# korrawe/harp

Measured on AMD Instinct MI355X. Metric: render+loss+backward+Adam frames/sec, 512x512 MANO hand mesh, higher is better.
Workload: dtype f32; 1 GPU; C3/C4: 256-frame 512x512 sequence, subdivided MANO hand 3093v/6152f/3327uv, self-shadow, coarse+appearance terms (displacement+texture stage, VGG excluded), dense Adam; global_batch=32, sequence_frames=256, hipgraph=True

## Files before the change

### harp_amd/csrc/raster.hip

```cpp
#include <stdlib.h>
#include <mutex>
#include <unordered_map>
#include "raster_body.h"

namespace {

using rb::Tri;

template <bool BITS>
__device__ __forceinline__ void face_setup_body(const float* __restrict__ ndc, const int32_t* __restrict__ faces,
                                                int V, int F, float r, FaceRec* __restrict__ recs,
                                                float4* __restrict__ bbs, int S, int nsx, unsigned long long* __restrict__ bits, int W64) {
  const int f = blockIdx.x * blockDim.x + threadIdx.x;
  const int b = blockIdx.y;
  float4 bb = make_float4(3.0e38f, -3.0e38f, 3.0e38f, -3.0e38f);
  if (f < F) {
    const FaceRec rec = rb::face_rec(ndc + (size_t)b * V * 3, faces, f, r);
    recs[(size_t)b * F + f] = rec;
    bbs[(size_t)b * F + f] = rec.bb;
    bb = rec.bb;
  }
  if constexpr (BITS) {
    const int lane = threadIdx.x & 63;
    const int chunk = f >> 6;
// ... 24 lines not shown
  face_setup_body<BITS>(ndc, faces, V, F, r, recs, bbs, S, nsx, bits, W64);
}

struct SetupView { const float* ndc; float r; RasterWs W; };

__global__ void __launch_bounds__(256) face_setup_pair_kernel(const SetupView a, const SetupView b, const int32_t* __restrict__ faces, int V, int F, int S) {
  const SetupView& v = blockIdx.z ? b : a;
  face_setup_body<true>(v.ndc, faces, V, F, v.r, v.W.recs, v.W.bbs, S, v.W.nsx, v.W.bits, v.W.W64);
}

__global__ void __launch_bounds__(256) bin_faces_kernel(const float4* __restrict__ bbs, int F, int S, int nsx,
                                                        int32_t* __restrict__ bins, int32_t* __restrict__ bin_count) {
  const int nst = nsx * nsx;
  const int st = blockIdx.x * 4 + (threadIdx.x >> 6), b = blockIdx.y;
  if (st >= nst) return;
  rb::bin_super_tile(bbs + (size_t)b * F, F, S, nsx, st, bins + ((size_t)b * nst + st) * F, bin_count + b * nst + st);
}

__device__ __forceinline__ void expand_bits_body(const unsigned long long* __restrict__ bits, int F, int W64, int nst,
                                                 int32_t* __restrict__ bins, int32_t* __restrict__ bin_count) {
  const int st = blockIdx.x * 4 + (threadIdx.x >> 6), b = blockIdx.y, lane = threadIdx.x & 63;
  if (st >= nst) return;
  const unsigned long long* src = bits + ((size_t)b * nst + st) * W64;
  int32_t* out = bins + ((size_t)b * nst + st) * F;
  int total = 0;
  for (int base = 0; base < W64; base += 128) {
    unsigned long long w0 = (base + lane < W64) ? src[base + lane] : 0ull;
    unsigned long long w1 = (base + 64 + lane < W64) ? src[base + 64 + lane] : 0ull;
    const int c0 = __popcll(w0), c1 = __popcll(w1);
    int incl = c0 | (c1 << 16);
#pragma unroll
    for (int o = 1; o < 64; o <<= 1) {
      const int t = __shfl_up(incl, o, 64);
      if (lane >= o) incl += t;
    }
    const int tot = __shfl(incl, 63, 64);
    int pos = total + (incl & 0xffff) - c0;
    const int f0 = (base + lane) * 64;
    while (w0) {
      out[pos++] = f0 + (int)__builtin_ctzll(w0);
      w0 &= w0 - 1ull;
    }
    pos = total + (tot & 0xffff) + (incl >> 16) - c1;
    while (w1) {
      out[pos++] = f0 + 4096 + (int)__builtin_ctzll(w1);
      w1 &= w1 - 1ull;
    }
    total += (tot & 0xffff) + (tot >> 16);
  }
  if (lane == 0) bin_count[b * nst + st] = total;
}
__global__ void __launch_bounds__(256) expand_bits_kernel(const unsigned long long* __restrict__ bits, int F, int W64, int nst,
                                                          int32_t* __restrict__ bins, int32_t* __restrict__ bin_count) {
  expand_bits_body(bits, F, W64, nst, bins, bin_count);
}
__global__ void __launch_bounds__(256) expand_bits_pair_kernel(const RasterWs a, const RasterWs b, int F) {
  const RasterWs& W = blockIdx.z ? b : a;
  expand_bits_body(W.bits, F, W.W64, W.nsx * W.nsx, W.bins, W.cnt);
}

__global__ void __launch_bounds__(1024) order_tiles_kernel(const int32_t* __restrict__ bin_count, int total, int32_t* __restrict__ order,
                                                           int32_t* __restrict__ nact) {
  __shared__ int s_hist[33], s_base[33];
  rb::order_tiles(bin_count, total, order, nact, s_hist, s_base);
}

__global__ void __launch_bounds__(1024) order_tiles_pair_kernel(const RasterWs a, const RasterWs b, int total) {
  __shared__ int s_hist[33], s_base[33];
  const RasterWs& W = blockIdx.x ? b : a;
  rb::order_tiles(W.cnt, total, W.order, W.nact, s_hist, s_base);
}

#ifndef RASTER_OCC1
#define RASTER_OCC1 7
#endif
#ifndef RASTER_OCC0
#define RASTER_OCC0 7
#endif
#ifndef RASTER_OCC2
#define RASTER_OCC2 8
#endif
constexpr unsigned kRasterGrid = 16384;

template <int MODE, bool LOOP, bool BWD = false>
__global__ void __launch_bounds__(256) __attribute__((amdgpu_waves_per_eu(MODE == 2 ? RASTER_OCC2 : (MODE == 0 ? RASTER_OCC0 : (BWD ? 5 : RASTER_OCC1)), 8))) raster_kernel(const FaceRec* __restrict__ recs, const float4* __restrict__ bbs,
                                                     const int32_t* __restrict__ bins,
                                                     const int32_t* __restrict__ bin_count, const int32_t* __restrict__ order,
                                                     const int32_t* __restrict__ nact, int B, int F, int S, int nsx,
                                                     float blur, float sigma, int32_t* __restrict__ face_id,
                                                     float* __restrict__ zbuf, float* __restrict__ alpha,
                                                     const float* __restrict__ g_alpha, const int32_t* __restrict__ faces,
                                                     int V, float* __restrict__ g_ndc, const float* __restrict__ l1_target,
                                                     const int32_t* __restrict__ l1_fid, const float* __restrict__ l1_w,
                                                     float* __restrict__ l1_loss, float* __restrict__ l1_grad, float l1_inv, int sparse,
                                                     const float* __restrict__ l1_bg_sums, int32_t* __restrict__ st_state,
                                                     uint32_t* __restrict__ srec, int srec_cap) {
  __shared__ rb::RasterSmem<MODE, BWD> sm;
  if constexpr (!LOOP) {
    rb::raster_tile<MODE, BWD>(sm, blockIdx.x, recs, bbs, bins, bin_count, order, nact, B, F, S, nsx, blur, sigma, face_id, zbuf, alpha, g_alpha, faces, V, g_ndc,
                          l1_target, l1_fid, l1_w, l1_loss, l1_grad, l1_inv, sparse, l1_bg_sums, st_state, srec, srec_cap);
    return;
  }
  const unsigned total = tile_grid(B, nsx);
  const int nst = nsx * nsx;
  const bool bg_table = (MODE == 1) && sparse && l1_target && l1_bg_sums;
  const bool skip_empty = (MODE == 2) || bg_table || (sparse && !zbuf && !(MODE == 1 && l1_target));
  const unsigned limit = skip_empty ? min(total, (unsigned)(((nact[0] + 7) / 8) * 8 * (kSuper / kTile) * (kSuper / kTile))) : total;
  for (unsigned v = blockIdx.x; v < limit; v += gridDim.x) {
    if (v != blockIdx.x) __syncthreads();
    rb::raster_tile<MODE, BWD>(sm, v, recs, bbs, bins, bin_count, order, nact, B, F, S, nsx, blur, sigma, face_id, zbuf, alpha, g_alpha, faces, V, g_ndc,
                          l1_target, l1_fid, l1_w, l1_loss, l1_grad, l1_inv, sparse, l1_bg_sums, st_state, srec, srec_cap);
  }
  if (bg_table) {
    float acc = 0.f;
    const int first = min(B * nst, (nact[0] + 7) / 8 * 8);
    for (int slot = first + (int)(blockIdx.x * blockDim.x + threadIdx.x); slot < B * nst; slot += (int)(gridDim.x * blockDim.x)) {
      const int entry = order[slot], b = entry / nst, st = entry - b * nst;
      acc += l1_bg_sums[(size_t)l1_fid[b] * nst + st];
    }
    if (acc != 0.f) atomicAdd(l1_loss, acc * l1_inv);
  }
}

}

extern "C" size_t harp_sil_records_bytes(int B, int S, int cap);
struct SilRecBinding { uint32_t* rec; int cap; size_t bytes; };
static std::mutex g_srec_mu;
static std::unordered_map<const void*, SilRecBinding> g_srec;
static SilRecBinding srec_of(const void* ws) {
  std::lock_guard<std::mutex> lk(g_srec_mu);
  const auto it = g_srec.find(ws);
  return it == g_srec.end() ? SilRecBinding{nullptr, 0, 0} : it->second;
}

static void raster_setup_any(const float* ndc, const int32_t* faces, int B, int V, int F, int S, float r, void* ws, hipStream_t stream) {
  const RasterWs W = raster_ws_split(ws, B, F, S);
  static const bool old_bins = [] { const char* e = getenv("HARP_BIN_SCAN"); return e && atoi(e) != 0; }();
  if (W.nsx <= 64 && !old_bins) {
    hipLaunchKernelGGL(face_setup_kernel<true>, dim3((F + 255) / 256, B), dim3(256), 0, stream, ndc, faces, V, F, r, W.recs, W.bbs, S, W.nsx, W.bits, W.W64);
    hipLaunchKernelGGL(expand_bits_kernel, dim3((W.nsx * W.nsx + 3) / 4, B), dim3(256), 0, stream, W.bits, F, W.W64, W.nsx * W.nsx, W.bins, W.cnt);
  } else {
    hipLaunchKernelGGL(face_setup_kernel<false>, dim3((F + 255) / 256, B), dim3(256), 0, stream, ndc, faces, V, F, r, W.recs, W.bbs, S, W.nsx, nullptr, 0);
    hipLaunchKernelGGL(bin_faces_kernel, dim3((W.nsx * W.nsx + 3) / 4, B), dim3(256), 0, stream, W.bbs, F, S, W.nsx, W.bins, W.cnt);
  }
  hipLaunchKernelGGL(order_tiles_kernel, dim3(1), dim3(1024), 0, stream, W.cnt, B * W.nsx * W.nsx, W.order, W.nact);
}

static unsigned raster_loop_grid(unsigned full_grid) {
  const char* e = getenv("HARP_RASTER_LOOP");
  if (e) {
    const int n = atoi(e);
    if (n <= 0) return 0u;
    return min(full_grid, (unsigned)((max(n, 8) + 7) / 8 * 8));
  }
  return full_grid > 65536u ? kRasterGrid : 0u;
}

int harp_detail_raster_setup(const float* ndc, const int32_t* faces, int B, int V, int F, int S, float r, void* ws, hipStream_t stream) {
  raster_setup_any(ndc, faces, B, V, F, S, r, ws, stream);
  HARP_CHECK_LAUNCH();
  return HARP_OK;
}

extern "C" {

size_t harp_rasterize_ws_bytes(int B, int F, int S) {
  const int nsx = (S + kSuper - 1) / kSuper;
  size_t recs = (size_t)B * F * sizeof(FaceRec);
  size_t bbs = (size_t)B * F * sizeof(float4);
  size_t bins = (size_t)B * nsx * nsx * F * sizeof(int32_t);
  size_t cnt = (((size_t)B * nsx * nsx * sizeof(int32_t)) + 255) / 256 * 256;
  size_t bits = (size_t)B * nsx * nsx * ((F + 63) / 64) * sizeof(unsigned long long);
  return recs + bbs + bins + 2 * cnt + 256 + bits;
}

static int rasterize_impl(const float* ndc, const int32_t* faces, int B, int V, int F, int S, int soft, float blur_radius,
                          float sigma, void* ws, int32_t* face_id, float* zbuf, float* alpha, const float* l1_target,
                          const int32_t* l1_fid, const float* l1_w, float* l1_loss, float* l1_grad, const float* l1_bg_sums,
                          int32_t* st_state, hipStream_t stream, float* g_ndc = nullptr) {
  if (!ndc || !faces || !ws || (!face_id && (!(soft & 1) || zbuf)) || B <= 0 || F <= 0 || S <= 0 || ((soft & 1) && !alpha)) return HARP_ERR_ARG;
  if (l1_target && (!(soft & 1) || !l1_fid || !l1_w || !l1_loss || !l1_grad)) return HARP_ERR_ARG;
  const RasterWs W = raster_ws_split(ws, B, F, S);
  FaceRec* recs = W.recs; int32_t *bins = W.bins, *cnt = W.cnt, *order = W.order; float4* bbs = W.bbs;
  const int nsx = W.nsx;
  const float r = (soft & 1) ? sqrtf(blur_radius) : 0.f;
  if (!(soft & 4)) raster_setup_any(ndc, faces, B, V, F, S, r, ws, stream);
  const unsigned lgrid = raster_loop_grid(tile_grid(B, nsx));
  const bool loop = lgrid != 0u;
  const dim3 grid(loop ? lgrid : tile_grid(B, nsx));
  const float l1_inv = 1.0f / ((float)B * (float)S * (float)S);
  const int sp = (soft & 2) ? 1 : 0;
#define HARP_RASTER_LAUNCH(MODE, LOOP, ...) hipLaunchKernelGGL((raster_kernel<MODE, LOOP>), grid, dim3(256), 0, stream, __VA_ARGS__)
  if ((soft & 1) && g_ndc) {
    if (loop) hipLaunchKernelGGL((raster_kernel<1, true, true>), grid, dim3(256), 0, stream, recs, bbs, bins, cnt, order, W.nact, B, F, S, nsx, blur_radius, sigma, face_id, zbuf,
                                 alpha, nullptr, faces, V, g_ndc, l1_target, l1_fid, l1_w, l1_loss, l1_grad, l1_inv, sp, l1_bg_sums, nullptr, nullptr, 0);
    else hipLaunchKernelGGL((raster_kernel<1, false, true>), grid, dim3(256), 0, stream, recs, bbs, bins, cnt, order, W.nact, B, F, S, nsx, blur_radius, sigma, face_id, zbuf,
                            alpha, nullptr, faces, V, g_ndc, l1_target, l1_fid, l1_w, l1_loss, l1_grad, l1_inv, sp, l1_bg_sums, nullptr, nullptr, 0);
  } else if (soft & 1) {
    const SilRecBinding sr = srec_of(ws);
    if (sr.rec && harp_sil_records_bytes(B, S, sr.cap) > sr.bytes) return HARP_ERR_ARG;
    uint32_t* srec = sr.rec;
    const int srec_cap = sr.cap;
    if (loop) HARP_RASTER_LAUNCH(1, true, recs, bbs, bins, cnt, order, W.nact, B, F, S, nsx, blur_radius, sigma, face_id, zbuf, alpha, nullptr, nullptr, 0, nullptr,
                                 l1_target, l1_fid, l1_w, l1_loss, l1_grad, l1_inv, sp, l1_bg_sums, nullptr, srec, srec_cap);
    else HARP_RASTER_LAUNCH(1, false, recs, bbs, bins, cnt, order, W.nact, B, F, S, nsx, blur_radius, sigma, face_id, zbuf, alpha, nullptr, nullptr, 0, nullptr,
                            l1_target, l1_fid, l1_w, l1_loss, l1_grad, l1_inv, sp, l1_bg_sums, nullptr, srec, srec_cap);
  } else {
    if (loop) HARP_RASTER_LAUNCH(0, true, recs, bbs, bins, cnt, order, W.nact, B, F, S, nsx, 0.f, 1.f, face_id, zbuf, nullptr, nullptr, nullptr, 0, nullptr, nullptr,
                                 nullptr, nullptr, nullptr, nullptr, 0.f, sp, nullptr, st_state, nullptr, 0);
    else HARP_RASTER_LAUNCH(0, false, recs, bbs, bins, cnt, order, W.nact, B, F, S, nsx, 0.f, 1.f, face_id, zbuf, nullptr, nullptr, nullptr, 0, nullptr, nullptr,
                            nullptr, nullptr, nullptr, nullptr, 0.f, sp, nullptr, st_state, nullptr, 0);
  }
  HARP_CHECK_LAUNCH();
  return HARP_OK;
}

int harp_raster_setup_pair(const float* ndc_a, float blur_radius_a, void* ws_a, const float* ndc_b, float blur_radius_b, void* ws_b,
                           const int32_t* faces, int B, int V, int F, int S, hipStream_t stream) {
  if (!ndc_a || !ndc_b || !ws_a || !ws_b || !faces || B <= 0 || V <= 0 || F <= 0 || S <= 0 || blur_radius_a < 0.f || blur_radius_b < 0.f) return HARP_ERR_ARG;
  SetupView a, b;
  a.ndc = ndc_a; a.r = sqrtf(blur_radius_a); a.W = raster_ws_split(ws_a, B, F, S);
  b.ndc = ndc_b; b.r = sqrtf(blur_radius_b); b.W = raster_ws_split(ws_b, B, F, S);
  if (a.W.nsx > 64) {
    raster_setup_any(ndc_a, faces, B, V, F, S, a.r, ws_a, stream);
    raster_setup_any(ndc_b, faces, B, V, F, S, b.r, ws_b, stream);
    HARP_CHECK_LAUNCH();
    return HARP_OK;
  }
  const int nst = a.W.nsx * a.W.nsx;
  hipLaunchKernelGGL(face_setup_pair_kernel, dim3((F + 255) / 256, B, 2), dim3(256), 0, stream, a, b, faces, V, F, S);
  hipLaunchKernelGGL(expand_bits_pair_kernel, dim3((nst + 3) / 4, B, 2), dim3(256), 0, stream, a.W, b.W, F);
  hipLaunchKernelGGL(order_tiles_pair_kernel, dim3(2), dim3(1024), 0, stream, a.W, b.W, B * nst);
  HARP_CHECK_LAUNCH();
  return HARP_OK;
}

int harp_rasterize_l1_fwd(const float* ndc, const int32_t* faces, int B, int V, int F, int S, int soft, float blur_radius,
                          float sigma, void* ws, int32_t* face_id, float* zbuf, float* alpha, const float* l1_target,
                          const int32_t* l1_fid, const float* l1_w, float* l1_loss, float* l1_grad, const float* l1_bg_sums,
                          hipStream_t stream) {
  return rasterize_impl(ndc, faces, B, V, F, S, soft, blur_radius, sigma, ws, face_id, zbuf, alpha, l1_target, l1_fid, l1_w, l1_loss, l1_grad,
                        l1_bg_sums, nullptr, stream);
}

int harp_rasterize_l1_fwd_bwd(const float* ndc, const int32_t* faces, int B, int V, int F, int S, int soft, float blur_radius,
                              float sigma, void* ws, int32_t* face_id, float* alpha, const float* l1_target, const int32_t* l1_fid,
                              const float* l1_w, float* l1_loss, float* l1_grad, const float* l1_bg_sums, float* g_ndc, hipStream_t stream) {
  if (!g_ndc || !l1_target || !(soft & 1)) return HARP_ERR_ARG;
  return rasterize_impl(ndc, faces, B, V, F, S, soft, blur_radius, sigma, ws, face_id, nullptr, alpha, l1_target, l1_fid, l1_w, l1_loss, l1_grad,
                        l1_bg_sums, nullptr, stream, g_ndc);
}

int harp_rasterize_fwd(const float* ndc, const int32_t* faces, int B, int V, int F, int S, int soft, float blur_radius,
                       float sigma, void* ws, int32_t* face_id, float* zbuf, float* alpha, hipStream_t stream) {
  return rasterize_impl(ndc, faces, B, V, F, S, soft, blur_radius, sigma, ws, face_id, zbuf, alpha, nullptr, nullptr, nullptr,
                        nullptr, nullptr, nullptr, nullptr, stream);
}

int harp_rasterize_fwd_keep(const float* ndc, const int32_t* faces, int B, int V, int F, int S, int sparse, void* ws, int32_t* face_id,
                            float* zbuf, int32_t* st_state, hipStream_t stream) {
  if (!zbuf || !st_state) return HARP_ERR_ARG;
  return rasterize_impl(ndc, faces, B, V, F, S, ((sparse & 3) ? 2 : 0) | (sparse & 4), 0.f, 1.f, ws, face_id, zbuf, nullptr, nullptr, nullptr, nullptr, nullptr,
                        nullptr, nullptr, st_state, stream);
}

int harp_silhouette_bwd(const int32_t* faces, int B, int V, int F, int S, float blur_radius, float sigma, const void* ws,
                        const float* alpha, const float* g_alpha, float* g_ndc, hipStream_t stream) {
  if (!faces || !ws || !alpha || !g_alpha || !g_ndc) return HARP_ERR_ARG;
  const SilRecBinding sr = srec_of(ws);
  if (sr.rec && harp_sil_records_bytes(B, S, sr.cap) > sr.bytes) return HARP_ERR_ARG;
  uint32_t* srec = sr.rec;
  const int srec_cap = sr.cap;
  const RasterWs W = raster_ws_split((void*)ws, B, F, S);
  FaceRec* recs = W.recs; int32_t *bins = W.bins, *cnt = W.cnt, *order = W.order; float4* bbs = W.bbs;
  const int nsx = W.nsx;
  const unsigned lgrid = raster_loop_grid(tile_grid(B, nsx));
  const bool loop = lgrid != 0u;
  const dim3 grid(loop ? lgrid : tile_grid(B, nsx));
  if (loop) HARP_RASTER_LAUNCH(2, true, recs, bbs, bins, cnt, order, W.nact, B, F, S, nsx, blur_radius, sigma, nullptr, nullptr, (float*)alpha, g_alpha, faces, V, g_ndc,
                               nullptr, nullptr, nullptr, nullptr, nullptr, 0.f, 0, nullptr, nullptr, srec, srec_cap);
  else HARP_RASTER_LAUNCH(2, false, recs, bbs, bins, cnt, order, W.nact, B, F, S, nsx, blur_radius, sigma, nullptr, nullptr, (float*)alpha, g_alpha, faces, V, g_ndc,
                          nullptr, nullptr, nullptr, nullptr, nullptr, 0.f, 0, nullptr, nullptr, srec, srec_cap);
  HARP_CHECK_LAUNCH();
  return HARP_OK;
}

size_t harp_sil_records_bytes(int B, int S, int cap) {
  if (B <= 0 || S <= 0 || cap < 0) return 0;
  const int nsx = (S + kSuper - 1) / kSuper;
  return (rb::srec_count_words(B, nsx) + rb::srec_tiles(B, nsx) * (size_t)cap) * sizeof(uint32_t);
}

int harp_sil_records_bind(const void* ws, void* sil_rec, int rec_cap, int B, int F, int S) {
// ... 10 lines not shown
```

### harp_amd/csrc/raster_body.h

```cpp
#pragma once
#include "harp_common.h"
#include "harp_hip.h"
#include <type_traits>

namespace rb {

constexpr int kStage = 256;

struct Tri {
  float x0, y0, z0, x1, y1, z1, x2, y2, z2;
};

__device__ __forceinline__ Tri tri_from(const float4 a, const float4 b, const float4 c) {
  Tri t;
  t.x0 = a.x; t.y0 = a.y; t.z0 = a.z; t.x1 = a.w;
  t.y1 = b.x; t.z1 = b.y; t.x2 = b.z; t.y2 = b.w;
  t.z2 = c.x;
  return t;
}

__device__ __forceinline__ bool tri_bary(const Tri& t, float px, float py, float& b0, float& b1, float& b2) {
  const float area = edge_fn(t.x2, t.y2, t.x0, t.y0, t.x1, t.y1) + kEps;
  const float w0 = edge_fn(px, py, t.x1, t.y1, t.x2, t.y2) / area;
  const float w1 = edge_fn(px, py, t.x2, t.y2, t.x0, t.y0) / area;
  const float w2 = edge_fn(px, py, t.x0, t.y0, t.x1, t.y1) / area;
  const float t0 = w0 * t.z1 * t.z2, t1 = t.z0 * w1 * t.z2, t2 = t.z0 * t.z1 * w2;
  const float den = fmaxf(t0 + t1 + t2, kEps);
  b0 = t0 / den; b1 = t1 / den; b2 = t2 / den;
  return b0 > 0.f && b1 > 0.f && b2 > 0.f;
}

__device__ __forceinline__ float seg_dist2(float px, float py, float ax, float ay, float bx, float by, float& tt) {
  const float bax = bx - ax, bay = by - ay;
  const float l2 = bax * bax + bay * bay;
  if (l2 <= kEps) { tt = 1.f; return (px - bx) * (px - bx) + (py - by) * (py - by); }
  float t = (bax * (px - ax) + bay * (py - ay)) * __builtin_amdgcn_rcpf(l2);
  t = fminf(fmaxf(t, 0.f), 1.f);
  tt = t;
  const float qx = ax + t * bax, qy = ay + t * bay;
  return (px - qx) * (px - qx) + (py - qy) * (py - qy);
}

__device__ __forceinline__ int block_compact(bool pred, int running, int* lds_cnt, int& total) {
  const unsigned long long m = __ballot(pred);
  const int lane = threadIdx.x & 63, w = threadIdx.x >> 6;
  if (lane == 0) lds_cnt[w] = __popcll(m);
  __syncthreads();
  int base = running;
  for (int i = 0; i < w; ++i) base += lds_cnt[i];
  total = lds_cnt[0] + lds_cnt[1] + lds_cnt[2] + lds_cnt[3];
  const int pos = base + __popcll(m & ((1ull << lane) - 1ull));
  __syncthreads();
  return pred ? pos : -1;
}

__device__ __forceinline__ int nst_of(int nsx) { return nsx * nsx; }

#ifndef RASTER_CAP2
#define RASTER_CAP2 128
#endif
template <int MODE> constexpr int stage_cap() { return MODE == 2 ? RASTER_CAP2 : kStage; }
template <int MODE, bool BWD = false>
struct RasterSmem {
  static constexpr int kCap = stage_cap<MODE>();
  float4 s_a[kCap], s_b[kCap], s_bb[kCap];
  float s_z2[MODE == 2 ? 1 : kCap];
  int32_t s_id[kCap];
  int lds_cnt[4];
  unsigned long long zkey[MODE <= 1 ? 256 : 1];
  int s_pre[MODE <= 1 ? kStage + 1 : 1];
  unsigned s_fb[MODE == 0 ? kStage : 1];
  typename std::conditional<BWD, int, unsigned char>::type sat[MODE == 1 ? 256 : 1];
  float prodl[MODE == 1 ? 256 : 1];
  unsigned char cand[MODE == 1 ? 256 : 1];
  float ndc_x[kTile], ndc_y[kTile];
  float rp_x[MODE == 2 ? 256 : 1], rp_y[MODE == 2 ? 256 : 1], rp_P[MODE == 2 ? 256 : 1], rp_g[MODE == 2 ? 256 : 1];
  alignas(4) unsigned short pairs[MODE >= 1 ? 512 : 1];
  double s_g[MODE == 2 ? kCap : 1][6];
  float s_gf[(MODE == 1 && BWD) ? kCap : 1][6];
  float red[4];
  int rec_n;
};

__device__ __forceinline__ void lds_add_f32(float* p, float v) {
  unsigned* u = reinterpret_cast<unsigned*>(p);
  unsigned old = *u, assumed;
  do {
    assumed = old;
    old = atomicCAS(u, assumed, __float_as_uint(__uint_as_float(assumed) + v));
  } while (old != assumed);
}

__host__ __device__ inline size_t srec_tiles(int B, int nsx) { return (size_t)B * nsx * nsx * ((kSuper / kTile) * (kSuper / kTile)); }
__host__ __device__ inline size_t srec_count_words(int B, int nsx) { return (srec_tiles(B, nsx) + 63) / 64 * 64; }

template <int MODE, bool BWD>
__device__ __forceinline__ void sil_bwd_records(RasterSmem<MODE, BWD>& sm, const uint32_t* __restrict__ rt, int nrec, int b, int tx0, int ty0,
                                                const FaceRec* __restrict__ rb, const int32_t* __restrict__ faces, int S, int V, float blur,
                                                float sigma, const float* __restrict__ alpha, const float* __restrict__ g_alpha,
                                                float* __restrict__ g_ndc) {
  static_assert(sizeof(VertexAccum<256, 2>) <= sizeof(sm.s_g), "vertex table must fit the face accumulators");
  auto* acc = reinterpret_cast<VertexAccum<256, 2>*>(&sm.s_g[0][0]);
  acc->clear();
  __syncthreads();
  const float inv_sigma = 1.0f / sigma;
  float* gb = g_ndc + (size_t)b * V * 3;
  for (int i = threadIdx.x; i < nrec; i += 256) {
    const unsigned rw = rt[i];
    const int c = (int)(rw & 255u), fid = (int)(rw >> 8);
    const int xi = tx0 + (c & (kTile - 1)), yi = ty0 + (c >> 4);
    const size_t o = ((size_t)b * S + yi) * S + xi;
    const float Pq = 1.0f - alpha[o], gq = g_alpha[o];
    if (Pq == 0.f || Pq == 1.0f || gq == 0.f) continue;
    const FaceRec fr = rb[fid];
    const int v0 = faces[3 * fid], v1 = faces[3 * fid + 1], v2 = faces[3 * fid + 2];
    const float qx = pix_to_ndc(xi, S), qy = pix_to_ndc(yi, S);
    const Tri t = tri_from(fr.a, fr.b, make_float4(0.f, 0.f, 0.f, 0.f));
    const float e0 = edge_fn(qx, qy, t.x1, t.y1, t.x2, t.y2);
    const float e1 = edge_fn(qx, qy, t.x2, t.y2, t.x0, t.y0);
    const float e2 = edge_fn(qx, qy, t.x0, t.y0, t.x1, t.y1);
    const float area = edge_fn(t.x2, t.y2, t.x0, t.y0, t.x1, t.y1) + kEps;
    const float sg = (area > 0.f) ? 1.f : ((area < 0.f) ? -1.f : 0.f);
    const float e0s = e0 * sg, e1s = e1 * sg, e2s = e2 * sg;
    const bool inside = (e0s > 0.f) && (e1s > 0.f) && (e2s > 0.f);
    const float l12 = (t.x2 - t.x1) * (t.x2 - t.x1) + (t.y2 - t.y1) * (t.y2 - t.y1);
    const float l20 = (t.x0 - t.x2) * (t.x0 - t.x2) + (t.y0 - t.y2) * (t.y0 - t.y2);
    const float l01 = (t.x1 - t.x0) * (t.x1 - t.x0) + (t.y1 - t.y0) * (t.y1 - t.y0);
    bool soft = true;
    if (inside) {
      const float K = 18.0f * sigma;
      if (e0 * e0 > K * l12 && e1 * e1 > K * l20 && e2 * e2 > K * l01) soft = false;
    } else {
      const float Bf = blur * 1.00001f;
      if ((e0s < 0.f && e0 * e0 >= Bf * l12) || (e1s < 0.f && e1 * e1 >= Bf * l20) || (e2s < 0.f && e2 * e2 >= Bf * l01)) soft = false;
    }
    if (!soft) continue;
    float ta, tb, tc;
    const float d01 = seg_dist2(qx, qy, t.x0, t.y0, t.x1, t.y1, ta);
    const float d02 = seg_dist2(qx, qy, t.x0, t.y0, t.x2, t.y2, tb);
    const float d12 = seg_dist2(qx, qy, t.x1, t.y1, t.x2, t.y2, tc);
    const float dist = fminf(d01, fminf(d02, d12));
    if (!(inside || dist < blur)) continue;
    const float sd = inside ? -dist : dist;
    const float p = __builtin_amdgcn_rcpf(1.0f + __expf(sd * inv_sigma));
    const float g_sd = gq * (-Pq * p * inv_sigma);
    const float gd = inside ? -g_sd : g_sd;
    int va, vb; float ax, ay, bx, by, tt;
    if (d01 <= d02 && d01 <= d12) { va = v0; vb = v1; ax = t.x0; ay = t.y0; bx = t.x1; by = t.y1; tt = ta; }
    else if (d02 <= d12)          { va = v0; vb = v2; ax = t.x0; ay = t.y0; bx = t.x2; by = t.y2; tt = tb; }
    else                          { va = v1; vb = v2; ax = t.x1; ay = t.y1; bx = t.x2; by = t.y2; tt = tc; }
    const float hx = ax + tt * (bx - ax), hy = ay + tt * (by - ay);
    const float cx = gd * 2.f * (hx - qx), cy = gd * 2.f * (hy - qy);
    const float gax = (1.f - tt) * cx, gay = (1.f - tt) * cy, gbx = tt * cx, gby = tt * cy;
    int k = acc->find(va);
    if (k >= 0) { acc->add(k, 0, gax); acc->add(k, 1, gay); }
    else { atomicAdd(gb + 3 * va, gax); atomicAdd(gb + 3 * va + 1, gay); }
    k = acc->find(vb);
    if (k >= 0) { acc->add(k, 0, gbx); acc->add(k, 1, gby); }
    else { atomicAdd(gb + 3 * vb, gbx); atomicAdd(gb + 3 * vb + 1, gby); }
  }
  __syncthreads();
  const int v = acc->key[threadIdx.x];
  if (v >= 0) {
    const float gx = (float)acc->val[threadIdx.x][0], gy = (float)acc->val[threadIdx.x][1];
    if (gx != 0.f) atomicAdd(gb + 3 * v, gx);
    if (gy != 0.f) atomicAdd(gb + 3 * v + 1, gy);
  }
}

template <int MODE, bool BWD = false>
__device__ __forceinline__ void raster_tile(RasterSmem<MODE, BWD>& sm, unsigned vblock, const FaceRec* __restrict__ recs, const float4* __restrict__ bbs,
                                                     const int32_t* __restrict__ bins,
                                                     const int32_t* __restrict__ bin_count, const int32_t* __restrict__ order,
                                                     const int32_t* __restrict__ nact, int B, int F, int S, int nsx,
                                                     float blur, float sigma, int32_t* __restrict__ face_id,
                                                     float* __restrict__ zbuf, float* __restrict__ alpha,
                                                     const float* __restrict__ g_alpha, const int32_t* __restrict__ faces,
                                                     int V, float* __restrict__ g_ndc, const float* __restrict__ l1_target,
                                                     const int32_t* __restrict__ l1_fid, const float* __restrict__ l1_w,
                                                     float* __restrict__ l1_loss, float* __restrict__ l1_grad, float l1_inv, int sparse,
                                                     const float* __restrict__ l1_bg_sums, int32_t* __restrict__ st_state = nullptr,
                                                     uint32_t* __restrict__ srec = nullptr, int srec_cap = 0) {
  auto& s_a = sm.s_a; auto& s_b = sm.s_b; auto& s_bb = sm.s_bb; auto& s_z2 = sm.s_z2; auto& s_id = sm.s_id;
  auto& s_g = sm.s_g;
  int* lds_cnt = sm.lds_cnt;

  int b, st, tx0, ty0, sub;
  const int kind = tile_decode_v(vblock, order, nact, B, nsx, S, b, st, tx0, ty0, sub, MODE != 2);
  if (kind == 0) return;
  if (kind == 2) {
    if (MODE == 2 || sub != 0) return;
    if (MODE == 0 && sparse && st_state && __syncthreads_or(st_state[b * nst_of(nsx) + st] == 1)) return;
    if (MODE == 1 && sparse && l1_target && l1_bg_sums) {
      if (threadIdx.x == 0) {
        const float sum = l1_bg_sums[(size_t)l1_fid[b] * nst_of(nsx) + st];
        if (sum != 0.f) atomicAdd(l1_loss, sum * l1_inv);
      }
      return;
    }
    float acc = 0.f;
    float tg[16];
    const bool l1 = (MODE == 1) && l1_target != nullptr;
    const float* trow = l1 ? l1_target + (size_t)l1_fid[b] * S * S : nullptr;
#pragma unroll
    for (int k = 0; k < 16; ++k) {
      int xi, yi;
      supertile_pixel(k, tx0, ty0, xi, yi);
      tg[k] = (l1 && xi < S && yi < S) ? trow[(size_t)yi * S + xi] : 0.f;
    }
#pragma unroll
    for (int k = 0; k < 16; ++k) {
      int xi, yi;
      supertile_pixel(k, tx0, ty0, xi, yi);
      if (xi < S && yi < S) {
        const size_t o = ((size_t)b * S + yi) * S + xi;
        if (l1) acc += fabsf(tg[k]);
        if (zbuf) zbuf[o] = -1.0f;
        if (!sparse) {
          if (face_id) face_id[o] = -1;
          if (MODE == 1) {
            alpha[o] = 0.f;
            if (l1) l1_grad[o] = l1_w[0] * l1_inv * (float)((0.f > tg[k]) - (0.f < tg[k]));
          }
        }
      }
    }
    if (MODE == 1 && l1_target) {
      const float sum = block_sum_256(acc, sm.red);
      if (threadIdx.x == 0 && sum != 0.f) atomicAdd(l1_loss, sum * l1_inv);
    }
    if (MODE == 0 && st_state && threadIdx.x == 0) st_state[b * nst_of(nsx) + st] = 1;
    return;
  }
  const int nst = nsx * nsx;
  if (MODE == 0 && st_state && sub == 0 && threadIdx.x == 0) st_state[b * nst + st] = 0;
  const unsigned rtile = (unsigned)((b * nst + st) * ((kSuper / kTile) * (kSuper / kTile)) + sub);
  const unsigned roff = (unsigned)srec_count_words(B, nsx) + rtile * (unsigned)srec_cap;
  if constexpr (MODE == 2) {
    if (srec != nullptr) {
      const int nrec = __builtin_amdgcn_readfirstlane(reinterpret_cast<const int32_t*>(srec)[rtile]);
      if (nrec <= srec_cap) {
        if (nrec > 0)
          sil_bwd_records(sm, srec + roff, nrec, b, tx0, ty0, recs + (size_t)b * F, faces, S, V,
                          blur, sigma, alpha, g_alpha, g_ndc);
        return;
      }
    }
  }
  const int lane = threadIdx.x & 63, w = threadIdx.x >> 6;
  const int xi = tx0 + (lane & 15), yi = ty0 + w * 4 + (lane >> 4);
  const bool in_img = (xi < S) && (yi < S);
  const float px = pix_to_ndc(xi, S), py = pix_to_ndc(yi, S);
  const int n = bin_count[b * nst + st];
  const int32_t* list = bins + ((size_t)b * nst + st) * F;
  const FaceRec* rb = recs + (size_t)b * F;
  const float4* bbb = bbs + (size_t)b * F;

  const float t_xhi = pix_to_ndc(tx0, S), t_xlo = pix_to_ndc(min(tx0 + kTile, S) - 1, S);
  const float t_yhi = pix_to_ndc(ty0, S), t_ylo = pix_to_ndc(min(ty0 + kTile, S) - 1, S);

  float best_z = 3.0e38f;
  int best_f = -1;
  float prod = 1.0f;
  float P = 0.f, ga = 0.f;
  bool need = in_img;
  if (MODE == 2) {
    if (in_img) {
      const size_t o = ((size_t)b * S + yi) * S + xi;
      P = 1.0f - alpha[o];
      ga = g_alpha[o];
    }
    need = in_img && (P != 0.f) && (P != 1.0f) && (ga != 0.f);
    if (__syncthreads_or(need ? 1 : 0) == 0) return;
  }
  constexpr bool kPix = (MODE == 2);
  int npx = 0;
  if constexpr (kPix) {
    const int slot = block_compact(need, 0, lds_cnt, npx);
    if (slot >= 0) { sm.rp_x[slot] = px; sm.rp_y[slot] = py; sm.rp_P[slot] = P; sm.rp_g[slot] = ga; }
  }

  const float inv_sigma = 1.0f / sigma;
  constexpr bool kScan = (MODE <= 1);
  if (kScan) {
    sm.zkey[threadIdx.x] = ~0ull;
    if (MODE == 1) { sm.sat[threadIdx.x] = 0; sm.prodl[threadIdx.x] = 1.0f; }
    if (MODE == 1 && threadIdx.x == 0) sm.rec_n = 0;
    if (threadIdx.x < kTile) sm.ndc_x[threadIdx.x] = pix_to_ndc(tx0 + threadIdx.x, S);
    else if (threadIdx.x < 2 * kTile) sm.ndc_y[threadIdx.x - kTile] = pix_to_ndc(ty0 + threadIdx.x - kTile, S);
  }
  auto stage_write = [&](int pos, int id, const float4& bb) {
    if (pos >= 0) {
      const FaceRec r = rb[id];
      s_a[pos] = r.a; s_b[pos] = r.b; s_bb[pos] = bb; s_id[pos] = id;
      if (MODE != 2) s_z2[pos] = r.c.x;
    }
  };
  int staged = 0, skip = 0;
  int rounds = 0, last_nl = 0;
  for (int base = 0; base < n || staged > 0;) {
    bool flush = true;
    if (base < n) {
      const int e = base + threadIdx.x;
      bool hit = false;
      int id = 0;
      float4 bb;
      if (e < n) {
        id = list[e];
        bb = bbb[id];
        hit = !(t_xlo > bb.y || t_xhi < bb.x || t_ylo > bb.w || t_yhi < bb.z);
      }
      int cnt;
      const int posc = block_compact(hit, 0, lds_cnt, cnt);
      const int rem = cnt - skip, room = stage_cap<MODE>() - staged;
      if (rem <= room) {
        stage_write((posc >= skip) ? staged + posc - skip : -1, id, bb);
        staged += rem;
        skip = 0;
        base += kStage;
        flush = base >= n;
      } else if (staged == 0) {
        stage_write((posc >= skip && posc < skip + room) ? posc - skip : -1, id, bb);
        staged = room;
        skip += room;
      }
    }
    if (!flush) continue;
    const int nl = staged;
    staged = 0;
    if (nl == 0) continue;
    ++rounds; last_nl = nl;
    if (MODE == 2) {
#pragma unroll
      for (int c = 0; c < 6; ++c)
        if ((int)threadIdx.x < stage_cap<MODE>()) s_g[threadIdx.x][c] = 0.0;
    }
    __syncthreads();
    if constexpr (kScan) {
      const float hs = 0.5f * (float)S;
      unsigned* s_fb = (MODE == 1) ? reinterpret_cast<unsigned*>(sm.pairs) : sm.s_fb;
      int nf, T;
      {
        int cnt = 0;
        unsigned box = 0;
        if ((int)threadIdx.x < nl) {
          const float4 q = s_bb[threadIdx.x];
          const int x0 = max((int)ceilf((1.0f - q.y) * hs - 0.501f), tx0), x1 = min(min((int)floorf((1.0f - q.x) * hs - 0.499f), tx0 + kTile - 1), S - 1);
          const int y0 = max((int)ceilf((1.0f - q.w) * hs - 0.501f), ty0), y1 = min(min((int)floorf((1.0f - q.z) * hs - 0.499f), ty0 + kTile - 1), S - 1);
          if (x0 <= x1 && y0 <= y1) {
            cnt = (x1 - x0 + 1) * (y1 - y0 + 1);
            box = (unsigned)(x0 - tx0) | ((unsigned)(y0 - ty0) << 4) | ((unsigned)(x1 - x0) << 8);
          }
        }
        const int own = cnt + ((cnt > 0) << 20);
        int v = own;
#pragma unroll
        for (int d = 1; d < 64; d <<= 1) {
          const int u = __shfl_up(v, d);
          if (lane >= d) v += u;
        }
        if (lane == 63) lds_cnt[w] = v;
        __syncthreads();
        int off = 0, tot = 0;
#pragma unroll
        for (int i = 0; i < 4; ++i) { const int c = lds_cnt[i]; tot += c; if (i < w) off += c; }
        const int excl = v + off - own;
        nf = tot >> 20; T = tot & 0xfffff;
        if (cnt > 0) {
          sm.s_pre[excl >> 20] = excl & 0xfffff;
          s_fb[excl >> 20] = threadIdx.x | (box << 8);
        }
        if (threadIdx.x == 0) sm.s_pre[nf] = T;
        __syncthreads();
      }
      if (T > 0) {
        const int per = (((T + 3) >> 2) + 63) & ~63;
        const int s_lo = w * per, s_end = min(T, s_lo + per);
        if (s_lo < s_end) {
          int kb = -1;
#pragma unroll
          for (int j = 0; j < kStage / 64; ++j) {
            const int idx = j * 64 + lane;
            kb += __popcll(__ballot(idx < nf && sm.s_pre[idx] <= s_lo));
          }
          int pkb = sm.s_pre[kb];
          const float K18 = 18.0f * sigma;
          for (int sb = s_lo; sb < s_end; sb += 64) {
            const int sl = sb + lane;
            const int pw = sm.s_pre[min(kb + 1 + lane, nf)];
            int k = kb, pk = pkb;
            const int lim = min(sb + 64, s_end);
            for (int j = 0; j < 64; ++j) {
              const int p = __builtin_amdgcn_readlane(pw, j);
              if (p >= lim) break;
              if (sl >= p) { ++k; pk = p; }
              ++kb; pkb = p;
            }
            if (sl < s_end) {
              const unsigned fb = s_fb[k];
              const int kk = fb & 255, wd = (int)((fb >> 16) & 15) + 1;
              const int r = sl - pk;
              const int ry = (int)(((float)r + 0.5f) * __builtin_amdgcn_rcpf((float)wd));
              const int xl = (int)((fb >> 8) & 15) + r - ry * wd, yl = (int)((fb >> 12) & 15) + ry;
              const float qx = sm.ndc_x[xl], qy = sm.ndc_y[yl];
              const float4 q = s_bb[kk];
              const Tri t = tri_from(s_a[kk], s_b[kk], make_float4(s_z2[kk], 0.f, 0.f, 0.f));
              const float area = edge_fn(t.x2, t.y2, t.x0, t.y0, t.x1, t.y1) + kEps;
              const float sg = (area > 0.f) ? 1.f : ((area < 0.f) ? -1.f : 0.f);
              const bool inbox = __builtin_amdgcn_fmed3f(qx, q.x, q.y) == qx && __builtin_amdgcn_fmed3f(qy, q.z, q.w) == qy;
// ... 157 lines not shown
          if (inside) {
            const float K = 18.0f * sigma;
            if (e0 * e0 > K * l12 && e1 * e1 > K * l20 && e2 * e2 > K * l01) soft = false;
          } else {
            const float Bf = blur * 1.00001f;
            if ((e0s < 0.f && e0 * e0 >= Bf * l12) || (e1s < 0.f && e1 * e1 >= Bf * l20) || (e2s < 0.f && e2 * e2 >= Bf * l01)) soft = false;
          }
          if (soft) {
            float ta, tb, tc;
            const float d01 = seg_dist2(qx, qy, t.x0, t.y0, t.x1, t.y1, ta);
            const float d02 = seg_dist2(qx, qy, t.x0, t.y0, t.x2, t.y2, tb);
            const float d12 = seg_dist2(qx, qy, t.x1, t.y1, t.x2, t.y2, tc);
            const float dist = fminf(d01, fminf(d02, d12));
            if (inside || dist < blur) {
              const float sd = inside ? -dist : dist;
              const float p = __builtin_amdgcn_rcpf(1.0f + __expf(sd * inv_sigma));
              const float g_sd = gq * (-Pq * p * inv_sigma);
              const float gd = inside ? -g_sd : g_sd;
              int ia, ib; float ax, ay, bx, by, tt;
              if (d01 <= d02 && d01 <= d12) { ia = 0; ib = 1; ax = t.x0; ay = t.y0; bx = t.x1; by = t.y1; tt = ta; }
              else if (d02 <= d12)          { ia = 0; ib = 2; ax = t.x0; ay = t.y0; bx = t.x2; by = t.y2; tt = tb; }
              else                          { ia = 1; ib = 2; ax = t.x1; ay = t.y1; bx = t.x2; by = t.y2; tt = tc; }
              const float hx = ax + tt * (bx - ax), hy = ay + tt * (by - ay);
              const float cx = gd * 2.f * (hx - qx), cy = gd * 2.f * (hy - qy);
              atomicAdd(&s_g[j][2 * ia], (double)((1.f - tt) * cx));
              atomicAdd(&s_g[j][2 * ia + 1], (double)((1.f - tt) * cy));
              atomicAdd(&s_g[j][2 * ib], (double)(tt * cx));
              atomicAdd(&s_g[j][2 * ib + 1], (double)(tt * cy));
            }
          }
        }
      };
      for (int i0 = w * per; i0 < i_end; i0 += 64) {
        const int i = i0 + lane;
        bool pass = false;
        int c = 0, k = 0;
        if (i < i_end) {
          c = (int)(((float)i + 0.5f) * inv_nl);
          k = i - c * nl;
          if (k < 0) { --c; k += nl; } else if (k >= nl) { ++c; k -= nl; }
          const float4 q = s_bb[k];
          const float qx = sm.rp_x[c], qy = sm.rp_y[c];
          pass = !(qx > q.y || qx < q.x || qy > q.w || qy < q.z);
        }
        const unsigned long long m = __ballot(pass);
        if (pass) wl[(tail + __popcll(m & ((1ull << lane) - 1ull))) & 127] = (unsigned short)((c << 8) | k);
        tail += __popcll(m);
        if (tail - head >= 64) { process(64); head += 64; }
      }
      if (tail > head) process(tail - head);
    }
    __syncthreads();
    if (MODE == 2 && (int)threadIdx.x < nl) {
      const int fid = s_id[threadIdx.x];
      float* gb = g_ndc + (size_t)b * V * 3;
#pragma unroll
      for (int k = 0; k < 3; ++k) {
        const float gx = (float)s_g[threadIdx.x][2 * k], gy = (float)s_g[threadIdx.x][2 * k + 1];
        if (gx != 0.f || gy != 0.f) {
          const int v = faces[3 * fid + k];
          atomicAdd(gb + 3 * v, gx);
          atomicAdd(gb + 3 * v + 1, gy);
        }
      }
    }
    __syncthreads();
  }

  if constexpr (kScan) {
    const unsigned long long key = sm.zkey[threadIdx.x];
    if (key != ~0ull) { best_f = (int)(unsigned)(key & 0xffffffffull); best_z = __uint_as_float((unsigned)(key >> 32)); }
    if (MODE == 1) prod = sm.sat[threadIdx.x] ? 0.f : sm.prodl[threadIdx.x];
    if (MODE == 1 && srec && threadIdx.x == 0) reinterpret_cast<int32_t*>(srec)[rtile] = sm.rec_n;
  }
  float l1_acc = 0.f;
  if (MODE != 2 && in_img) {
    const size_t o = ((size_t)b * S + yi) * S + xi;
    if (face_id) face_id[o] = best_f;
    if (zbuf) zbuf[o] = (best_f >= 0) ? best_z : -1.0f;
    if (MODE == 1) {
      const float a = 1.0f - prod;
      alpha[o] = a;
      if (l1_target) {
        const float d = a - l1_target[((size_t)l1_fid[b] * S + yi) * S + xi];
        l1_acc = fabsf(d);
        l1_grad[o] = l1_w[0] * l1_inv * ((d > 0.f) - (d < 0.f));
      }
    }
  }
  if (MODE == 1 && l1_target) {
    const float sum = block_sum_256(l1_acc, sm.red);
    if (threadIdx.x == 0 && sum != 0.f) atomicAdd(l1_loss, sum * l1_inv);
  }
  if constexpr (MODE == 1 && BWD) {
    if (g_ndc != nullptr && l1_target != nullptr) {
      float Pq = 0.f, gq = 0.f;
      if (in_img) {
        const float a = 1.0f - prod;
        const float d = a - l1_target[((size_t)l1_fid[b] * S + yi) * S + xi];
        Pq = 1.0f - a;
        gq = l1_w[0] * l1_inv * ((d > 0.f) - (d < 0.f));
      }
      const bool rim = in_img && (Pq != 0.f) && (Pq != 1.0f) && (gq != 0.f);
      if (__syncthreads_or(rim ? 1 : 0) != 0) {
        float* rp_x = reinterpret_cast<float*>(sm.zkey);
        float* rp_y = rp_x + 256;
        float* rp_P = reinterpret_cast<float*>(sm.sat);
        float* rp_g = sm.prodl;
        int npx;
        const int slot = block_compact(rim, 0, lds_cnt, npx);
        if (slot >= 0) { rp_x[slot] = px; rp_y[slot] = py; rp_P[slot] = Pq; rp_g[slot] = gq; }
        auto bwd_round = [&](int nl) {
#pragma unroll
          for (int c = 0; c < 6; ++c) sm.s_gf[threadIdx.x][c] = 0.f;
          __syncthreads();
          const int npairs = npx * nl;
          const float inv_nl = 1.0f / (float)nl;
          unsigned short* wl = sm.pairs + w * 128;
          const int per = (npairs + 3) >> 2, i_end = min(npairs, (w + 1) * per);
          int head = 0, tail = 0;
          auto process = [&](int nvalid) {
            if (lane < nvalid) {
              const int pr = wl[(head + lane) & 127], c = pr >> 8, j = pr & 255;
              const float qx = rp_x[c], qy = rp_y[c], Pc = rp_P[c], gc = rp_g[c];
              const Tri t = tri_from(s_a[j], s_b[j], make_float4(0.f, 0.f, 0.f, 0.f));
              const float e0 = edge_fn(qx, qy, t.x1, t.y1, t.x2, t.y2);
              const float e1 = edge_fn(qx, qy, t.x2, t.y2, t.x0, t.y0);
              const float e2 = edge_fn(qx, qy, t.x0, t.y0, t.x1, t.y1);
              const float area = edge_fn(t.x2, t.y2, t.x0, t.y0, t.x1, t.y1) + kEps;
              const float sg = (area > 0.f) ? 1.f : ((area < 0.f) ? -1.f : 0.f);
              const float e0s = e0 * sg, e1s = e1 * sg, e2s = e2 * sg;
              const bool inside = (e0s > 0.f) && (e1s > 0.f) && (e2s > 0.f);
              const float l12 = (t.x2 - t.x1) * (t.x2 - t.x1) + (t.y2 - t.y1) * (t.y2 - t.y1);
              const float l20 = (t.x0 - t.x2) * (t.x0 - t.x2) + (t.y0 - t.y2) * (t.y0 - t.y2);
              const float l01 = (t.x1 - t.x0) * (t.x1 - t.x0) + (t.y1 - t.y0) * (t.y1 - t.y0);
              bool soft = true;
              if (inside) {
                const float K = 18.0f * sigma;
                if (e0 * e0 > K * l12 && e1 * e1 > K * l20 && e2 * e2 > K * l01) soft = false;
              } else {
                const float Bf = blur * 1.00001f;
                if ((e0s < 0.f && e0 * e0 >= Bf * l12) || (e1s < 0.f && e1 * e1 >= Bf * l20) || (e2s < 0.f && e2 * e2 >= Bf * l01)) soft = false;
              }
              if (soft) {
                float ta, tb, tc;
                const float d01 = seg_dist2(qx, qy, t.x0, t.y0, t.x1, t.y1, ta);
                const float d02 = seg_dist2(qx, qy, t.x0, t.y0, t.x2, t.y2, tb);
                const float d12 = seg_dist2(qx, qy, t.x1, t.y1, t.x2, t.y2, tc);
                const float dist = fminf(d01, fminf(d02, d12));
                if (inside || dist < blur) {
                  const float sd = inside ? -dist : dist;
                  const float p = __builtin_amdgcn_rcpf(1.0f + __expf(sd * inv_sigma));
                  const float g_sd = gc * (-Pc * p * inv_sigma);
                  const float gd = inside ? -g_sd : g_sd;
                  int ia, ib; float ax, ay, bx, by, tt;
                  if (d01 <= d02 && d01 <= d12) { ia = 0; ib = 1; ax = t.x0; ay = t.y0; bx = t.x1; by = t.y1; tt = ta; }
                  else if (d02 <= d12)          { ia = 0; ib = 2; ax = t.x0; ay = t.y0; bx = t.x2; by = t.y2; tt = tb; }
                  else                          { ia = 1; ib = 2; ax = t.x1; ay = t.y1; bx = t.x2; by = t.y2; tt = tc; }
                  const float hx = ax + tt * (bx - ax), hy = ay + tt * (by - ay);
                  const float cx = gd * 2.f * (hx - qx), cy = gd * 2.f * (hy - qy);
                  lds_add_f32(&sm.s_gf[j][2 * ia], (1.f - tt) * cx);
                  lds_add_f32(&sm.s_gf[j][2 * ia + 1], (1.f - tt) * cy);
                  lds_add_f32(&sm.s_gf[j][2 * ib], tt * cx);
                  lds_add_f32(&sm.s_gf[j][2 * ib + 1], tt * cy);
                }
              }
            }
          };
          for (int i0 = w * per; i0 < i_end; i0 += 64) {
            const int i = i0 + lane;
            bool pass = false;
            int c = 0, k = 0;
            if (i < i_end) {
              c = (int)(((float)i + 0.5f) * inv_nl);
              k = i - c * nl;
              if (k < 0) { --c; k += nl; } else if (k >= nl) { ++c; k -= nl; }
              const float4 q = s_bb[k];
              const float qx = rp_x[c], qy = rp_y[c];
              pass = !(qx > q.y || qx < q.x || qy > q.w || qy < q.z);
            }
            const unsigned long long m = __ballot(pass);
            if (pass) wl[(tail + __popcll(m & ((1ull << lane) - 1ull))) & 127] = (unsigned short)((c << 8) | k);
            tail += __popcll(m);
            if (tail - head >= 64) { process(64); head += 64; }
// ... 148 lines not shown
```

Measured before the change: 53570 frames/s.

## Stage four bin entries per thread and prefetch L1 targets in raster tiles

The raster tile kernel gains a compile-time KS parameter. With KS=4, each thread loads four face ids with one vector load, culls them against the tile bounding box, and compacts hits through per-wave ballots, so one round can consume several 256-entry chunks of the bin list. Face ids and the L1 silhouette target are now fetched before the bin count and parked in LDS to hide global latency. The cost is more registers and LDS. The L1 value is only written to LDS inside the staging loop, so a tile with an empty bin list may read an unwritten LDS slot. K=4 is the default for the non-loop forward launches, while the backward and loop paths stay at K=1.

```diff
diff --git a/harp_amd/csrc/raster.hip b/harp_amd/csrc/raster.hip
--- a/harp_amd/csrc/raster.hip
+++ b/harp_amd/csrc/raster.hip
@@ -130,7 +130,7 @@
 #endif
 constexpr unsigned kRasterGrid = 16384;
 
-template <int MODE, bool LOOP, bool BWD = false>
+template <int MODE, bool LOOP, bool BWD = false, int K = 1>
 __global__ void __launch_bounds__(256) __attribute__((amdgpu_waves_per_eu(MODE == 2 ? RASTER_OCC2 : (MODE == 0 ? RASTER_OCC0 : (BWD ? 5 : RASTER_OCC1)), 8))) raster_kernel(const FaceRec* __restrict__ recs, const float4* __restrict__ bbs,
                                                      const int32_t* __restrict__ bins,
                                                      const int32_t* __restrict__ bin_count, const int32_t* __restrict__ order,
@@ -145,7 +145,7 @@
                                                      uint32_t* __restrict__ srec, int srec_cap) {
   __shared__ rb::RasterSmem<MODE, BWD> sm;
   if constexpr (!LOOP) {
-    rb::raster_tile<MODE, BWD>(sm, blockIdx.x, recs, bbs, bins, bin_count, order, nact, B, F, S, nsx, blur, sigma, face_id, zbuf, alpha, g_alpha, faces, V, g_ndc,
+    rb::raster_tile<MODE, BWD, K>(sm, blockIdx.x, recs, bbs, bins, bin_count, order, nact, B, F, S, nsx, blur, sigma, face_id, zbuf, alpha, g_alpha, faces, V, g_ndc,
                           l1_target, l1_fid, l1_w, l1_loss, l1_grad, l1_inv, sparse, l1_bg_sums, st_state, srec, srec_cap);
     return;
   }
@@ -156,7 +156,7 @@
   const unsigned limit = skip_empty ? min(total, (unsigned)(((nact[0] + 7) / 8) * 8 * (kSuper / kTile) * (kSuper / kTile))) : total;
   for (unsigned v = blockIdx.x; v < limit; v += gridDim.x) {
     if (v != blockIdx.x) __syncthreads();
-    rb::raster_tile<MODE, BWD>(sm, v, recs, bbs, bins, bin_count, order, nact, B, F, S, nsx, blur, sigma, face_id, zbuf, alpha, g_alpha, faces, V, g_ndc,
+    rb::raster_tile<MODE, BWD, K>(sm, v, recs, bbs, bins, bin_count, order, nact, B, F, S, nsx, blur, sigma, face_id, zbuf, alpha, g_alpha, faces, V, g_ndc,
                           l1_target, l1_fid, l1_w, l1_loss, l1_grad, l1_inv, sparse, l1_bg_sums, st_state, srec, srec_cap);
   }
   if (bg_table) {
@@ -203,6 +203,18 @@
     return min(full_grid, (unsigned)((max(n, 8) + 7) / 8 * 8));
   }
   return full_grid > 65536u ? kRasterGrid : 0u;
+}
+
+#ifndef RASTER_STAGE_K
+#define RASTER_STAGE_K 4
+#endif
+static int raster_stage_k(bool loop) {
+  const char* e = getenv("HARP_RASTER_STAGE_K");
+  if (e) {
+    const int k = atoi(e);
+    if (k == 1 || k == 4) return k;
+  }
+  return loop ? 1 : RASTER_STAGE_K;
 }
 
 int harp_detail_raster_setup(const float* ndc, const int32_t* faces, int B, int V, int F, int S, float r, void* ws, hipStream_t stream) {
@@ -240,6 +252,12 @@
   const float l1_inv = 1.0f / ((float)B * (float)S * (float)S);
   const int sp = (soft & 2) ? 1 : 0;
 #define HARP_RASTER_LAUNCH(MODE, LOOP, ...) hipLaunchKernelGGL((raster_kernel<MODE, LOOP>), grid, dim3(256), 0, stream, __VA_ARGS__)
+#define HARP_RASTER_LAUNCH_K(MODE, LOOP, ...)                                                                            \
+  do {                                                                                                                   \
+    if (stage_k == 4) hipLaunchKernelGGL((raster_kernel<MODE, LOOP, false, 4>), grid, dim3(256), 0, stream, __VA_ARGS__); \
+    else hipLaunchKernelGGL((raster_kernel<MODE, LOOP, false, 1>), grid, dim3(256), 0, stream, __VA_ARGS__);              \
+  } while (0)
+  const int stage_k = raster_stage_k(loop);
   if ((soft & 1) && g_ndc) {
     if (loop) hipLaunchKernelGGL((raster_kernel<1, true, true>), grid, dim3(256), 0, stream, recs, bbs, bins, cnt, order, W.nact, B, F, S, nsx, blur_radius, sigma, face_id, zbuf,
                                  alpha, nullptr, faces, V, g_ndc, l1_target, l1_fid, l1_w, l1_loss, l1_grad, l1_inv, sp, l1_bg_sums, nullptr, nullptr, 0);
@@ -250,14 +268,14 @@
     if (sr.rec && harp_sil_records_bytes(B, S, sr.cap) > sr.bytes) return HARP_ERR_ARG;
     uint32_t* srec = sr.rec;
     const int srec_cap = sr.cap;
-    if (loop) HARP_RASTER_LAUNCH(1, true, recs, bbs, bins, cnt, order, W.nact, B, F, S, nsx, blur_radius, sigma, face_id, zbuf, alpha, nullptr, nullptr, 0, nullptr,
+    if (loop) HARP_RASTER_LAUNCH_K(1, true, recs, bbs, bins, cnt, order, W.nact, B, F, S, nsx, blur_radius, sigma, face_id, zbuf, alpha, nullptr, nullptr, 0, nullptr,
                                  l1_target, l1_fid, l1_w, l1_loss, l1_grad, l1_inv, sp, l1_bg_sums, nullptr, srec, srec_cap);
-    else HARP_RASTER_LAUNCH(1, false, recs, bbs, bins, cnt, order, W.nact, B, F, S, nsx, blur_radius, sigma, face_id, zbuf, alpha, nullptr, nullptr, 0, nullptr,
+    else HARP_RASTER_LAUNCH_K(1, false, recs, bbs, bins, cnt, order, W.nact, B, F, S, nsx, blur_radius, sigma, face_id, zbuf, alpha, nullptr, nullptr, 0, nullptr,
                             l1_target, l1_fid, l1_w, l1_loss, l1_grad, l1_inv, sp, l1_bg_sums, nullptr, srec, srec_cap);
   } else {
-    if (loop) HARP_RASTER_LAUNCH(0, true, recs, bbs, bins, cnt, order, W.nact, B, F, S, nsx, 0.f, 1.f, face_id, zbuf, nullptr, nullptr, nullptr, 0, nullptr, nullptr,
+    if (loop) HARP_RASTER_LAUNCH_K(0, true, recs, bbs, bins, cnt, order, W.nact, B, F, S, nsx, 0.f, 1.f, face_id, zbuf, nullptr, nullptr, nullptr, 0, nullptr, nullptr,
                                  nullptr, nullptr, nullptr, nullptr, 0.f, sp, nullptr, st_state, nullptr, 0);
-    else HARP_RASTER_LAUNCH(0, false, recs, bbs, bins, cnt, order, W.nact, B, F, S, nsx, 0.f, 1.f, face_id, zbuf, nullptr, nullptr, nullptr, 0, nullptr, nullptr,
+    else HARP_RASTER_LAUNCH_K(0, false, recs, bbs, bins, cnt, order, W.nact, B, F, S, nsx, 0.f, 1.f, face_id, zbuf, nullptr, nullptr, nullptr, 0, nullptr, nullptr,
                             nullptr, nullptr, nullptr, nullptr, 0.f, sp, nullptr, st_state, nullptr, 0);
   }
   HARP_CHECK_LAUNCH();
diff --git a/harp_amd/csrc/raster_body.h b/harp_amd/csrc/raster_body.h
--- a/harp_amd/csrc/raster_body.h
+++ b/harp_amd/csrc/raster_body.h
@@ -80,6 +80,7 @@
   float s_gf[(MODE == 1 && BWD) ? kCap : 1][6];
   float red[4];
   int rec_n;
+  float l1_y[MODE == 1 ? 256 : 1];
 };
 
 __device__ __forceinline__ void lds_add_f32(float* p, float v) {
@@ -168,7 +169,7 @@
   }
 }
 
-template <int MODE, bool BWD = false>
+template <int MODE, bool BWD = false, int KS = 1>
 __device__ __forceinline__ void raster_tile(RasterSmem<MODE, BWD>& sm, unsigned vblock, const FaceRec* __restrict__ recs, const float4* __restrict__ bbs,
                                                      const int32_t* __restrict__ bins,
                                                      const int32_t* __restrict__ bin_count, const int32_t* __restrict__ order,
@@ -251,10 +252,37 @@
   const int xi = tx0 + (lane & 15), yi = ty0 + w * 4 + (lane >> 4);
   const bool in_img = (xi < S) && (yi < S);
   const float px = pix_to_ndc(xi, S), py = pix_to_ndc(yi, S);
-  const int n = bin_count[b * nst + st];
+  static_assert(KS == 1 || KS == 2 || KS == 4, "a sub-chunk of 256 list entries must be a whole number of waves");
+  static_assert(KS == 1 || (MODE <= 1 && !BWD), "the backward forms stage one entry per thread");
   const int32_t* list = bins + ((size_t)b * nst + st) * F;
   const FaceRec* rb = recs + (size_t)b * F;
   const float4* bbb = bbs + (size_t)b * F;
+  int ids[KS];
+  auto load_ids = [&](int base) {
+    const int e0 = base + KS * (int)threadIdx.x;
+    if constexpr (KS > 1) {
+      using IdVec = typename std::conditional<KS == 4, int4, int2>::type;
+      if (base + KS * kStage <= F && (reinterpret_cast<uintptr_t>(list + base) & (sizeof(IdVec) - 1)) == 0) {
+        const IdVec v = *reinterpret_cast<const IdVec*>(list + e0);
+        ids[0] = v.x; ids[1] = v.y;
+        if constexpr (KS == 4) { ids[2] = v.z; ids[3] = v.w; }
+        return;
+      }
+    }
+#pragma unroll
+    for (int j = 0; j < KS; ++j) ids[j] = list[min(e0 + j, F - 1)];
+  };
+  bool ids_loaded = MODE != 2;
+  if (MODE != 2) load_ids(0);
+  const int n = bin_count[b * nst + st];
+  float l1_y = 0.f, l1_wt = 0.f;
+  if (MODE == 1 && l1_target) {
+    l1_wt = l1_w[0];
+    if (in_img) l1_y = l1_target[((size_t)l1_fid[b] * S + yi) * S + xi];
+  }
+  auto park_l1 = [&](bool first_pass) {
+    if (MODE == 1 && first_pass && l1_target) sm.l1_y[threadIdx.x] = l1_y;
+  };
 
   const float t_xhi = pix_to_ndc(tx0, S), t_xlo = pix_to_ndc(min(tx0 + kTile, S) - 1, S);
   const float t_yhi = pix_to_ndc(ty0, S), t_ylo = pix_to_ndc(min(ty0 + kTile, S) - 1, S);
@@ -301,30 +329,109 @@
   for (int base = 0; base < n || staged > 0;) {
     bool flush = true;
     if (base < n) {
-      const int e = base + threadIdx.x;
-      bool hit = false;
-      int id = 0;
-      float4 bb;
-      if (e < n) {
-        id = list[e];
-        bb = bbb[id];
-        hit = !(t_xlo > bb.y || t_xhi < bb.x || t_ylo > bb.w || t_yhi < bb.z);
-      }
-      int cnt;
-      const int posc = block_compact(hit, 0, lds_cnt, cnt);
-      const int rem = cnt - skip, room = stage_cap<MODE>() - staged;
-      if (rem <= room) {
-        stage_write((posc >= skip) ? staged + posc - skip : -1, id, bb);
-        staged += rem;
-        skip = 0;
-        base += kStage;
-        flush = base >= n;
-      } else if (staged == 0) {
-        stage_write((posc >= skip && posc < skip + room) ? posc - skip : -1, id, bb);
-        staged = room;
-        skip += room;
-      }
-    }
+      const bool first_pass = base == 0 && rounds == 0;
+      if (!ids_loaded) load_ids(base);
+      ids_loaded = false;
+      if constexpr (KS == 1) {
+        const int e = base + threadIdx.x;
+        bool hit = false;
+        const int id = (e < n) ? ids[0] : 0;
+        float4 bb;
+        if (e < n) {
+          bb = bbb[id];
+        }
+        park_l1(first_pass);
+        if (e < n) hit = !(t_xlo > bb.y || t_xhi < bb.x || t_ylo > bb.w || t_yhi < bb.z);
+        int cnt;
+        const int posc = block_compact(hit, 0, lds_cnt, cnt);
+        const int rem = cnt - skip, room = stage_cap<MODE>() - staged;
+        if (rem <= room) {
+          stage_write((posc >= skip) ? staged + posc - skip : -1, id, bb);
+          staged += rem;
+          skip = 0;
+          base += kStage;
+          flush = base >= n;
+        } else if (staged == 0) {
+          stage_write((posc >= skip && posc < skip + room) ? posc - skip : -1, id, bb);
+          staged = room;
+          skip += room;
+        }
+      } else {
+        constexpr int kWps = 4 / KS;
+        const int e0 = base + KS * (int)threadIdx.x;
+        float4 bb[KS];
+        bool hit[KS];
+#pragma unroll
+        for (int j = 0; j < KS; ++j) {
+          if (e0 + j >= n) ids[j] = 0;
+          bb[j] = bbb[ids[j]];
+        }
+        park_l1(first_pass);
+        const unsigned long long lt = (1ull << lane) - 1ull;
+        int below = 0, wtot = 0;
+#pragma unroll
+        for (int j = 0; j < KS; ++j) {
+          hit[j] = (e0 + j < n) && !(t_xlo > bb[j].y || t_xhi < bb[j].x || t_ylo > bb[j].w || t_yhi < bb[j].z);
+          const unsigned long long m = __ballot(hit[j]);
+          below += __popcll(m & lt);
+          wtot += __popcll(m);
+        }
+        if (lane == 0) lds_cnt[w] = wtot;
+        __syncthreads();
+        int wc[4];
+#pragma unroll
+        for (int i = 0; i < 4; ++i) wc[i] = lds_cnt[i];
+        __syncthreads();
+        const int sj = w / kWps;
+#pragma unroll
+        for (int i = 0; i < 4; ++i)
+          if (i / kWps == sj && i < w) below += wc[i];
+        const int staged0 = staged;
+        int my_lo = 0, my_hi = 0, my_off = 0;
+        int adv = 0;
+        bool stop = false;
+#pragma unroll
+        for (int j = 0; j < KS; ++j) {
+          if (stop || base + j * kStage >= n) continue;
+          int c = 0;
+#pragma unroll
+          for (int i = 0; i < kWps; ++i) c += wc[j * kWps + i];
+          const int rem = c - skip, room = stage_cap<MODE>() - staged;
+          int lo = 0, hi = 0, off = 0;
+          if (rem <= room) {
+            lo = skip; hi = c; off = staged - skip;
+            staged += rem;
+            skip = 0;
+            ++adv;
+          } else if (staged == 0) {
+            lo = skip; hi = skip + room; off = -skip;
+            staged = room;
+            skip += room;
+            stop = true;
+          } else {
+            stop = true;
+          }
+          if (sj == j) { my_lo = lo; my_hi = hi; my_off = off; }
+        }
+        base += adv * kStage;
+        flush = stop || base >= n;
+#pragma unroll
+        for (int j = 0; j < KS; ++j) {
+          if (hit[j] && below >= my_lo && below < my_hi) s_id[my_off + below] = ids[j];
+          below += hit[j] ? 1 : 0;
+        }
+        __syncthreads();
+        const int slot = staged0 + (int)threadIdx.x;
+        if (slot < staged) {
+          const FaceRec* r = rb + s_id[slot];
+          const float4 ra = r->a, rbv = r->b, rbb = r->bb;
+          const float rz = r->c.x;
+          s_a[slot] = ra; s_b[slot] = rbv; s_bb[slot] = rbb; s_z2[slot] = rz;
+        }
+      }
+    }
+#pragma unroll
+    for (int j = 0; j < KS; ++j) ids[j] = 0;
     if (!flush) continue;
     const int nl = staged;
     staged = 0;
@@ -648,9 +755,9 @@
       const float a = 1.0f - prod;
       alpha[o] = a;
       if (l1_target) {
-        const float d = a - l1_target[((size_t)l1_fid[b] * S + yi) * S + xi];
+        const float d = a - sm.l1_y[threadIdx.x];
         l1_acc = fabsf(d);
-        l1_grad[o] = l1_w[0] * l1_inv * ((d > 0.f) - (d < 0.f));
+        l1_grad[o] = l1_wt * l1_inv * ((d > 0.f) - (d < 0.f));
       }
     }
   }
@@ -663,9 +770,9 @@
       float Pq = 0.f, gq = 0.f;
       if (in_img) {
         const float a = 1.0f - prod;
-        const float d = a - l1_target[((size_t)l1_fid[b] * S + yi) * S + xi];
+        const float d = a - sm.l1_y[threadIdx.x];
         Pq = 1.0f - a;
-        gq = l1_w[0] * l1_inv * ((d > 0.f) - (d < 0.f));
+        gq = l1_wt * l1_inv * ((d > 0.f) - (d < 0.f));
       }
       const bool rim = in_img && (Pq != 0.f) && (Pq != 1.0f) && (gq != 0.f);
       if (__syncthreads_or(rim ? 1 : 0) != 0) {
```

Result: no change. 53890 frames/s, median of 3 (+0.6%).
